# Lynne-Zheng-Linfang/HS-Pose

Hardware: AMD Instinct MI355X
Metric: point-clouds/sec (N=1028) HS-layer fwd+bwd (higher is better)
Workload: dtype f32; 1 GPU; HS stack (FaceRecon backbone -> feat) fwd+bwd, B=16/GPU N=1028 fp32, train-mode BN, random-init weights (BASELINE configs[1] shape); global_batch=16, points=1028, parallelism=dp1, hipgraph=True, split_graph=False, grad_exchange=none

## Files before the change

### hs_pose_amd/FaceRecon.py

```python
import os

import torch
import torch.nn as nn
import torch.nn.functional as F

from . import gcn3d, ops, ops_bf16, pc_sample
from .config import FLAGS


def _conv_bn_relu_rows(seq, x, n_blocks, first=None):
    if (x.dtype if x is not None else getattr(first, "dtype", None)) == torch.bfloat16:
        for i in range(n_blocks):
            conv, bn = seq[3 * i], seq[3 * i + 1]
            x = first if (i == 0 and first is not None) else ops_bf16.dense_bn(x, conv.weight.squeeze(-1), conv.bias, bn)
        return x
    for i in range(n_blocks):
        conv, bn = seq[3 * i], seq[3 * i + 1]
        y, part = first if (i == 0 and first is not None) else ops.linear_rows(x, conv.weight.squeeze(-1), conv.bias, bn_partials=True)
        x = ops.bn_relu(y, bn, partial=part)
    return x


class FaceRecon(nn.Module):

# ... 69 lines not shown
                 (w(self.face_head[6]), True, True), (w(self.face_head[9]), True, False)]
        return specs

    def forward(self, vertices: "tensor (bs, vetice_num, 3)", cat_id: "tensor (bs, 1)"):
        bs, vertice_num, _ = vertices.size()
        k = self.neighbor_num
        if self._x3 is None:
            self._x3 = ops.X3Planes()
        exact = (not self.training or self.exact_train) and self.feature_dtype == torch.float32
        with ops.x3_scope(self._x3), ops.exact_scope(exact), pc_sample.draw_scope(None, vertices.device):
            return self._forward(vertices, cat_id)

    def _forward(self, vertices, cat_id):
        bs, vertice_num, _ = vertices.size()
        k = self.neighbor_num
        if self._bf16 is not None:
            self._bf16.refresh()
        else:
            ops.x3_refresh()
        with gcn3d.knn_scope():
            up = (gcn3d.prefetch_levels(vertices, k, self.pool_1.neighbor_num, rates=(self.pool_1.pooling_rate, self.pool_2.pooling_rate),
                                        samplers=(self.pool_1.sampler, self.pool_2.sampler))
                  if self.pool_1.neighbor_num == self.pool_2.neighbor_num else None)
            od = self.feature_dtype if self.feature_dtype == torch.bfloat16 else None
            fork0 = od is None and not self.keep_backward_cut and torch.is_grad_enabled()
            if fork0:
                fm_0, a_0 = self.conv_0(vertices, k, relu_fork=True)
            else:
                fm_0 = F.relu(self.conv_0(vertices, k), inplace=True)
            fork = od is None and not self.keep_backward_cut

            def layer_bn(conv, bn, *a):
                if od is None and bn.training and bn.track_running_stats and torch.is_grad_enabled() and not ops.exact_forward():
                    out, part = conv(*a, bn_shift=True)
                    return ops.bn_relu(out, bn, fork=fork, partial=part)
                if conv is self.conv_3 and ops.exact_forward():
                    return ops.bn_relu(conv(*a, transposed_view=True), bn, out_dtype=od, fork=fork)
                return ops.bn_relu(conv(*a), bn, out_dtype=od, fork=fork)
# ... 52 lines not shown
```

### hs_pose_amd/csrc/common.h

```cpp
#pragma once
#include <hip/hip_runtime.h>
#include <stdint.h>
#include <limits.h>
#include <math.h>

#include "hsp.h"

#define HSP_WAVE 64
#define HSP_NUM_XCD 8
#define HSP_NUM_CU 256

namespace hsp {

void set_last_hip_error(hipError_t e);

inline int check_launch() {
    hipError_t e = hipGetLastError();
    if (e != hipSuccess) {
        set_last_hip_error(e);
        return HSP_ERR_LAUNCH;
    }
    return HSP_OK;
}

inline hipStream_t as_stream(hspStream_t s) { return reinterpret_cast<hipStream_t>(s); }

template <typename... P, typename... A>
inline int launch_lds(void (*kern)(P...), dim3 grid, dim3 block, size_t lds, hipStream_t st, A... args) {
    if (lds > 64 * 1024) {
        hipError_t e = hipFuncSetAttribute(reinterpret_cast<const void*>(kern), hipFuncAttributeMaxDynamicSharedMemorySize, (int)lds);
        if (e != hipSuccess) { set_last_hip_error(e); return HSP_ERR_LAUNCH; }
    }
    hipLaunchKernelGGL(kern, grid, block, lds, st, args...);
    return check_launch();
}

int knn_feat_select_flags(const float* x, int B, int N, int C, int k, int drop, int quad_mode, int32_t* idx, void* ws, size_t ws_bytes,
                          uint8_t* tie, float* dmat, hspStream_t stream);
int knn3_select_flags(const float* x, int B, int N, int k, int drop, int k2, int32_t* idx, int32_t* idx2, uint8_t* tie,
                      hipStream_t st, bool* needs_tie_pass);

int colsum_cloud_plan(int B, int N, int C, int* rows, int* nchunk);

bool orl_exact_shape_ok(int N, int C);
#define HSP_BN_MAX_PARTIALS 512
bool gemm_wave_takes(const HspGemmCall& c);
bool gemm_rows_takes(const HspGemmCall& c);

inline bool al16(const void* q, long long ld, int es) { return ((reinterpret_cast<size_t>(q) | ((size_t)ld * es)) & 15) == 0; }

inline int persistent_blocks(long long work_items, int blocks_per_cu) {
    long long g = (long long)HSP_NUM_CU * blocks_per_cu;
    if (work_items < g) g = ((work_items + HSP_NUM_XCD - 1) / HSP_NUM_XCD) * HSP_NUM_XCD;
    if (g < HSP_NUM_XCD) g = HSP_NUM_XCD;
    return (int)g;
// ... 75 lines not shown
```

### hs_pose_amd/csrc/gemm_x3.hip

```cpp
#include "common.h"
#include <stdlib.h>
#include <type_traits>

namespace hsp {

using f32x16 = __attribute__((ext_vector_type(16))) float;
using bf16x8 = __attribute__((ext_vector_type(8))) __bf16;
using u32x4 = __attribute__((ext_vector_type(4))) unsigned;

struct X3Args {
    const float* A[2];
    const unsigned short* P[2];
    int lda[2], ldp[2], K[2];
    long long ps[2];
    float* C; int ldc;
    int M, N;
    const float* bias;
    const float* resid; int ldr;
    const float* cbias; int rpc;
    float alpha;
    int tiles_m, tiles_n, nsplit;
    float* ws;
    float* bn_shift;
    float* bn_part;
// ... 441 lines not shown
            const long long row = e / N4;
            const int c4 = (int)(e - row * N4);
            *reinterpret_cast<float4*>(C + (size_t)row * ldc + 4 * c4) = make_float4(alpha * s.x, alpha * s.y, alpha * s.z, alpha * s.w);
        }
    } else {
        for (long long e = (long long)blockIdx.x * 256 + threadIdx.x; e < total; e += (long long)gridDim.x * 256) {
            float s = ws[e];
            for (int sp = 1; sp < nsplit; ++sp) s += ws[(size_t)sp * total + e];
            const long long row = e / N;
            C[(size_t)row * ldc + (int)(e - row * N)] = alpha * s;
        }
    }
}

__global__ __launch_bounds__(256) void split_params_x3_kernel(const HspSplitDesc* __restrict__ tab, int n) {
    __shared__ float tile[64][33];
    int e = 0;
    while (e + 1 < n && (int)blockIdx.x >= tab[e + 1].tile0) ++e;
    const HspSplitDesc d = tab[e];
    const int t = (int)blockIdx.x - d.tile0;
    const int Nn = d.transpose ? d.cols : d.rows, Kk = d.transpose ? d.rows : d.cols;
    const int tk = (Kk + 63) >> 6;
    const int n0 = (t / tk) * 32, k0 = (t % tk) * 64;
    const int lx = threadIdx.x & 31, ly = threadIdx.x >> 5;
    unsigned* dst = reinterpret_cast<unsigned*>(d.dst);
    float x0[4], x1[4];
    if (d.transpose) {
#pragma unroll
        for (int j = 0; j < 8; ++j) {
            const int k = k0 + ly + 8 * j, nn = n0 + lx;
            tile[ly + 8 * j][lx] = (k < Kk && nn < Nn) ? d.src[(size_t)k * d.ld + nn] : 0.f;
        }
        __syncthreads();
#pragma unroll
        for (int j = 0; j < 4; ++j) { x0[j] = tile[2 * lx][ly + 8 * j]; x1[j] = tile[2 * lx + 1][ly + 8 * j]; }
    } else {
#pragma unroll
        for (int j = 0; j < 4; ++j) {
            const int nn = n0 + ly + 8 * j, k = k0 + 2 * lx;
            const float* p = d.src + (size_t)min(nn, Nn - 1) * d.ld;
            x0[j] = (nn < Nn && k < Kk) ? p[k] : 0.f;
            x1[j] = (nn < Nn && k + 1 < Kk) ? p[k + 1] : 0.f;
        }
    }
#pragma unroll
    for (int j = 0; j < 4; ++j) {
        const int nn = n0 + ly + 8 * j, k = k0 + 2 * lx;
        if (nn >= Nn || k >= Kk) continue;
        float r1[2], r2[2];
        const float xs[2] = {x0[j], x1[j]};
#pragma unroll
        for (int q = 0; q < 2; ++q) {
            const float h = __uint_as_float(__float_as_uint(xs[q]) & 0xffff0000u);
            r1[q] = xs[q] - h;
            const float m = __uint_as_float(__float_as_uint(r1[q]) & 0xffff0000u);
            r2[q] = r1[q] - m;
        }
        const size_t o = ((size_t)nn * d.kp + k) >> 1;
        const size_t psd = (size_t)d.ps >> 1;
        dst[o] = __builtin_amdgcn_perm(__float_as_uint(xs[1]), __float_as_uint(xs[0]), 0x07060302u);
        dst[psd + o] = __builtin_amdgcn_perm(__float_as_uint(r1[1]), __float_as_uint(r1[0]), 0x07060302u);
        dst[2 * psd + o] = __builtin_amdgcn_perm(__float_as_uint(r2[1]), __float_as_uint(r2[0]), 0x07060302u);
    }
}

static int x3_pick_split(long long tiles, int TT) {
    constexpr int per_cu = 2;
    if (tiles >= 2 * HSP_NUM_CU || TT < 16) return 1;
    int ns = (int)((per_cu * HSP_NUM_CU + tiles - 1) / tiles);
    if (ns > TT / 8) ns = TT / 8;
    if (ns > 16) ns = 16;
    if (ns < 2) return 1;
    const int per = (TT + ns - 1) / ns;
    return (TT + per - 1) / per;
}

static int x3_pick_wm(int M, int N) {
    const long long t128 = (long long)((M + 127) / 128) * ((N + X3_BN - 1) / X3_BN);
// ... 504 lines not shown
```

### hs_pose_amd/csrc/knn.hip

```cpp
#include "knn_common.h"
#include "tie_pass.h"
#include <float.h>
#include <type_traits>

namespace hsp {

using f32x16 = __attribute__((ext_vector_type(16))) float;

template <int K1>
struct TopList {
    float d[K1];
    int i[K1];
    __device__ __forceinline__ void init() {
#pragma unroll
        for (int p = 0; p < K1; ++p) { d[p] = INFINITY; i[p] = INT_MAX; }
    }
    __device__ __forceinline__ void insert(float v, int idx) {
        if (v < d[K1 - 1]) {
            bool lt_cur = true;
#pragma unroll
            for (int p = K1 - 1; p > 0; --p) {
                const bool lt_prev = v < d[p - 1];
                i[p] = lt_prev ? i[p - 1] : (lt_cur ? idx : i[p]);
                d[p] = __builtin_amdgcn_fmed3f(d[p - 1], d[p], v);
// ... 296 lines not shown
                }
            }
        }
        __builtin_amdgcn_wave_barrier();
    }
}

template <int S>
__global__ __launch_bounds__(256) void knn3_wave_kernel(const float* __restrict__ x, int N, int k, int drop,
                                                        int32_t* __restrict__ idx, int msel, uint8_t* __restrict__ tie,
                                                        int msel2, int32_t* __restrict__ idx2, int k2, int tie_inline, int QW) {
    extern __shared__ __attribute__((aligned(16))) char smem[];
    const int b = blockIdx.y;
    knn3_wave_body<S>(smem, x + (size_t)b * N * 3, nullptr, nullptr, nullptr, N, k, drop, idx, msel, tie, msel2, idx2, k2, tie_inline,
                      (size_t)b * N, (int)blockIdx.x, QW);
}

template <int W>
__device__ __forceinline__ void multi_row_sum(const float* __restrict__ row, long long size, float (&out)[4][W]) {
    int lp = 0;
    {
        long long v = 1; int r = 0;
        while (v < size) { v <<= 1; ++r; }
        lp = r / 4;
        if (lp < 4) lp = 4;
    }
    const long long level_step = 1ll << lp, level_mask = level_step - 1;
    float acc[4][4][W];
#pragma unroll
    for (int a = 0; a < 4; ++a)
// ... 886 lines not shown
        default: return HSP_ERR_UNSUPPORTED;
    }
}

template <int K1, int T>
static int launch_knn3(const float* x, int B, int N, int k, int drop, int32_t* idx, hipStream_t st, int msel, uint8_t* tie,
                       int msel2, int32_t* idx2, int k2) {
    const int chunk = N < 4096 ? N : 4096;
    size_t lds = (size_t)chunk * 16;
    if (lds < (size_t)256 * K1 * 8) lds = (size_t)256 * K1 * 8;
    constexpr int Q = 256 / T;
    return launch_lds(knn3_kernel<K1, T>, dim3((N + Q - 1) / Q, B), dim3(256), lds, st, x, N, k, drop, idx, chunk, msel, tie, msel2, idx2,
                      k2);
}

static int knn3_wave_tie_inline(int N) { return N <= 64 * 9 ? 1 : 0; }

template <int S>
static int launch_knn3_wave(const float* x, int B, int N, int k, int drop, int32_t* idx, hipStream_t st, int msel, uint8_t* tie,
                            int msel2, int32_t* idx2, int k2) {
    const int tie_inline = tie ? knn3_wave_tie_inline(N) : 0;
    const size_t lds = (size_t)N * 16 + (size_t)4 * KNN3W_SV * 8 + 4 * 64 * 4 +
                       (tie_inline ? (size_t)16 * N * 4 : 0);
    const int QW = (long long)B * N >= 8192 ? KNN3W_QW : 1;
    return launch_lds(knn3_wave_kernel<S>, dim3((N + 4 * QW - 1) / (4 * QW), B), dim3(256), lds, st, x, N, k, drop, idx, msel, tie, msel2,
                      idx2, k2, tie_inline, QW);
}

template <int K1>
static int launch_knn3_t(const float* x, int B, int N, int k, int drop, int32_t* idx, hipStream_t st, int msel = 0,
                         uint8_t* tie = nullptr, int msel2 = 0, int32_t* idx2 = nullptr, int k2 = 0) {
    const long long nq = (long long)B * N;
    if (N >= 64 && (nq < 131072 || N > 64 * 17)) {
        if (N <= 64 * 5) return launch_knn3_wave<5>(x, B, N, k, drop, idx, st, msel, tie, msel2, idx2, k2);
        if (N <= 64 * 9) return launch_knn3_wave<9>(x, B, N, k, drop, idx, st, msel, tie, msel2, idx2, k2);
        if (N <= 64 * 17) return launch_knn3_wave<17>(x, B, N, k, drop, idx, st, msel, tie, msel2, idx2, k2);
        if (N <= 64 * 33) return launch_knn3_wave<33>(x, B, N, k, drop, idx, st, msel, tie, msel2, idx2, k2);
        if (N <= 64 * 65) return launch_knn3_wave<65>(x, B, N, k, drop, idx, st, msel, tie, msel2, idx2, k2);
    }
    if (nq >= 131072) return launch_knn3<K1, 1>(x, B, N, k, drop, idx, st, msel, tie, msel2, idx2, k2);
    if (nq >= 32768) return launch_knn3<K1, 4>(x, B, N, k, drop, idx, st, msel, tie, msel2, idx2, k2);
    return launch_knn3<K1, 16>(x, B, N, k, drop, idx, st, msel, tie, msel2, idx2, k2);
}

enum { KF_REM_TILE = 0,
       KF_REM_WG = 1,
       KF_REM_SYM = 2 };

static size_t knn_feat_lds(int C, int K1) {
    const int Cp = (C + 63) & ~63;
    const size_t lds = (size_t)(32 * (Cp + 4) + 4 * 32 * KF_CT_STRIDE + 4 * 32 + 32 * 8) * 4;
    const size_t lds_lists = (size_t)256 * K1 * 8;
    return lds_lists > lds ? lds_lists : lds;
}
// ... 171 lines not shown
    merge_write<K1, 2>(lists, src, ml, k, drop, ovalid, idx + ((size_t)b * N + (ovalid ? oq : 0)) * k, N, ovalid ? oq : 0);
}

template <int K1>
static int launch_knn_feat_bf16(const bf16_t* x, const float* quad, int B, int N, int C, int k, int drop, int32_t* idx,
                                hipStream_t st) {
    if (C > 256) return HSP_ERR_UNSUPPORTED;
    size_t lds = (size_t)(128 + 64) * (C * 2 + 16) + (size_t)(4 * 16 * 64 + 2 * 32 + 128 * 2) * 4;
    const size_t lds_lists = (size_t)256 * K1 * 8;
    if (lds_lists > lds) lds = lds_lists;
    if (lds > 160 * 1024) return HSP_ERR_UNSUPPORTED;
    return launch_lds(knn_feat_bf16_kernel<K1>, dim3((N + 127) / 128, B), dim3(256), lds, st, x, quad, N, C, k, drop, idx);
}

int knn3_select_flags(const float* x, int B, int N, int k, int drop, int k2, int32_t* idx, int32_t* idx2, uint8_t* tie,
                      hipStream_t st, bool* needs_tie_pass) {
    *needs_tie_pass = !(N >= 64 && (long long)B * N < 131072 && knn3_wave_tie_inline(N) != 0);
    const int m = k + drop;
    const int msel = m + 1 < N ? m + 1 : N;
    const int msel2 = k2 > 0 ? k2 + drop + 1 : 0;
    return dispatch_k1(pick_k1(msel), [&](auto K) { return launch_knn3_t<K()>(x, B, N, k, drop, idx, st, msel, tie, msel2, idx2, k2); });
}

}

using namespace hsp;

#ifdef HSP_KNN_PROF
extern "C" int hsp_debug_set_knn_prof(void* dev_buf) {
    return hipMemcpyToSymbol(HIP_SYMBOL(hsp::g_knn_prof), &dev_buf, sizeof(void*)) == hipSuccess ? 0 : -1;
}
#endif

extern "C" size_t hsp_knn_workspace_bytes(int B, int N, int C, int k) {
    (void)k;
    if (C == 3 || B <= 0 || N <= 0) return 0;
// ... 118 lines not shown
                                       int k1, int kpool, int k2, int drop_first, float* v1, float* v2, int32_t* idx1,
                                       int32_t* idx1_pool, int32_t* idx2, int32_t* up1, int32_t* up2, hspStream_t stream) {
    if (!xyz || !sel1 || !sel2 || !v1 || !v2 || !idx1 || !idx2 || !up1 || !up2 || B <= 0 || N0 <= 0 || k1 <= 0 || k2 <= 0 || kpool < 0 ||
        (kpool > 0) != (idx1_pool != nullptr) || kpool > k1)
        return HSP_ERR_BAD_ARG;
    if (!hsp_geometry_levels_takes(N0, N1, N2, k1, kpool, k2, drop_first)) return HSP_ERR_UNSUPPORTED;
    return geometry_impl(xyz, B, N0, sel1, N1, sel2, N2, k1, kpool, k2, drop_first ? 1 : 0, v1, v2, idx1, idx1_pool, idx2, up1, up2, nullptr,
                         0, 0, nullptr, nullptr, as_stream(stream));
}

extern "C" size_t hsp_geometry_all_workspace_bytes(int B, int N0) {
    if (B <= 0 || N0 <= 0) return 0;
    return ((size_t)B * N0 + 255) & ~(size_t)255;
}

extern "C" int hsp_geometry_all_f32(const float* xyz, int B, int N0, int k0, int kpool0, const int32_t* sel1, int N1,
                                    const int32_t* sel2, int N2, int k1, int kpool, int k2, int drop_first, int32_t* idx0,
                                    int32_t* idx0_pool, float* v1, float* v2, int32_t* idx1, int32_t* idx1_pool, int32_t* idx2,
                                    int32_t* up1, int32_t* up2, void* ws, size_t ws_bytes, hspStream_t stream) {
    if (!xyz || !sel1 || !sel2 || !v1 || !v2 || !idx0 || !idx1 || !idx2 || !up1 || !up2 || B <= 0 || N0 <= 0 || k0 <= 0 || k1 <= 0 ||
        k2 <= 0 || kpool < 0 || kpool0 < 0 || (kpool > 0) != (idx1_pool != nullptr) || (kpool0 > 0) != (idx0_pool != nullptr) ||
        kpool > k1 || kpool0 > k0)
        return HSP_ERR_BAD_ARG;
    const int drop = drop_first ? 1 : 0;
    if (!hsp_geometry_all_takes(B, N0, k0, kpool0, N1, N2, k1, kpool, k2, drop_first)) return HSP_ERR_UNSUPPORTED;
    if (!ws || ws_bytes < hsp_geometry_all_workspace_bytes(B, N0)) return HSP_ERR_WORKSPACE;
    uint8_t* tie = reinterpret_cast<uint8_t*>(ws);
    bool needs_pass = true;
    int rc = knn3_select_flags(xyz, B, N0, k0, drop, kpool0, idx0, idx0_pool, tie, as_stream(stream), &needs_pass);
    if (rc) return rc;
    if (!needs_pass) return HSP_ERR_UNSUPPORTED;
    return geometry_impl(xyz, B, N0, sel1, N1, sel2, N2, k1, kpool, k2, drop, v1, v2, idx1, idx1_pool, idx2, up1, up2, tie, k0, kpool0,
                         idx0, idx0_pool, as_stream(stream));
}

extern "C" int hsp_nn1_f32(const float* tgt, int Nt, const float* src, int Ns, int B, int32_t* idx,
                           hspStream_t stream) {
    if (!tgt || !src || !idx || B <= 0 || Nt <= 0 || Ns <= 0) return HSP_ERR_BAD_ARG;
    const size_t lds = (size_t)Ns * 16;
    if (lds > 160 * 1024) return HSP_ERR_UNSUPPORTED;
    return launch_lds(nn1_kernel, dim3((Nt + 255) / 256, B), dim3(256), lds, as_stream(stream), tgt, Nt, src, Ns, idx);
}
```

### hs_pose_amd/gcn3d.py

```python
import contextlib
import math

import torch
import torch.nn as nn
import torch.nn.functional as F

from . import ops, pc_sample
from .config import FLAGS

_knn_memo = None


POOL_K = 4


@contextlib.contextmanager
def knn_scope():
    global _knn_memo, _levels
    prev, _knn_memo = _knn_memo, {}
    prev_levels, _levels = _levels, None
    try:
        yield
    finally:
        _knn_memo, _levels = prev, prev_levels
# ... 26 lines not shown
    n2 = int(n1 / 4)
    k1, k2 = min(k, n1 // 8), min(k, n2 // 8)
    if (vertices.shape[2] != 3 or n2 < 1 or k1 < 1 or k2 < 1 or k1 + 1 > n1 or k2 + 1 > n2
            or not ops._takes("hsp_fps_levels_takes", n0)):
        return None
    sel1, v1, v2 = ops.fps_levels(vertices, n1, n2)
    _xyz_knn(v1, k1)
    if pool_k != POOL_K or k1 <= POOL_K:
        _xyz_knn(v1, pool_k)
    _xyz_knn(v2, k2)
    _levels = {id(vertices): (vertices, sel1, v1), id(v1): (v1, torch.arange(n2, dtype=torch.int32, device=vertices.device), v2),
               "up": (ops.nn1(vertices, v1), ops.nn1(vertices, v2))}
    return _levels["up"]


def prefetch_levels(vertices, k, pool_k=None, rates=(4, 4), samplers=(None, None)):
    global _levels
    _levels = None
    if _knn_memo is None or vertices.dtype != torch.float32 or vertices.requires_grad or not vertices.is_cuda:
        return None
    pool_k = POOL_K if pool_k is None else pool_k
    how = {resolve_sampler(s_) for s_ in samplers}
    if how != {"random"}:
        return _prefetch_levels_fps(vertices, k, pool_k) if how == {"fps"} and tuple(rates) == (4, 4) else None
    B, n0, C = vertices.shape
    n1 = int(n0 / 4)
    n2 = int(n1 / 4)
    k1, k2 = min(k, n1 // 8), min(k, n2 // 8)
    with_input = k > pool_k and ops.geometry_all_takes(B, n0, C, k, pool_k, n1, n2, k1, pool_k, k2)
    if tuple(rates) != (4, 4) or k1 <= pool_k or not (with_input or ops.geometry_levels_takes(n0, C, n1, n2, k1, pool_k, k2)):
        return None
    if _pool_feed is not None:
        sel1, sel2 = next(_pool_feed), next(_pool_feed)
        assert sel1.numel() == n1 and sel2.numel() == n2 and sel1.dtype == torch.int32
    else:
        with pc_sample.draw_scope(None, vertices.device) as device_draws:
            if device_draws is not None:
                sel1, sel2 = device_draws.pool_rows(n0, 4, levels=2)
            else:
                sel1 = torch.randperm(n0)[:n1].to(device=vertices.device, dtype=torch.int32)
                sel2 = torch.randperm(n1)[:n2].to(device=vertices.device, dtype=torch.int32)
    if with_input:
        geo = ops.geometry_all(vertices, k, pool_k, sel1, sel2, k1, pool_k, k2)
        _knn_memo[id(vertices)] = (vertices, {k: geo["idx0"], pool_k: geo["idx0_pool"]})
    else:
        geo = ops.geometry_levels(vertices, sel1, sel2, k1, pool_k, k2)
    v1, v2 = geo["v1"], geo["v2"]
    _knn_memo[id(v1)] = (v1, {k1: geo["idx1"], pool_k: geo["idx1_pool"]})
    _knn_memo[id(v2)] = (v2, {k2: geo["idx2"]})
    _levels = {id(vertices): (vertices, sel1, v1), id(v1): (v1, sel2, v2), "up": (geo["up1"], geo["up2"])}
    return _levels["up"]


def _xyz_knn(vertices, k):
    if _knn_memo is None or vertices.dtype != torch.float32:
        return ops.knn(vertices, k)
    key = id(vertices)
    hit = _knn_memo.get(key)
# ... 192 lines not shown
```

### hs_pose_amd/ops.py

```python
import ctypes
import functools
import os

import torch

from ._lib import (BATCH_SELECT_MAX_ITEMS, BATCH_SELECT_MAX_SEGS, ERR_UNSUPPORTED, FOLD_MAX_DIRS, FOLD_MAX_WGRAD, HspDirsPending, HspError,
                   HspGemmCall, HspSelectSeg, HspSplitDesc, HspWgradPending, check, lib)
from ._lib import (GEMM_BN_LINEAR as BN_LINEAR, GEMM_BN_OUT as BN_OUT, GEMM_ROUTE_SMALL_ROWS as ROUTE_SMALL_ROWS, GEMM_ROUTE_TILE as ROUTE_TILE,
                   GEMM_ROUTE_WAVE as ROUTE_WAVE, GEMM_ROUTE_X3 as ROUTE_X3, GEMM_ROUTE_X3_BN as ROUTE_X3_BN)

from .config import FLAGS

_vp = ctypes.c_void_p

DETERMINISTIC = os.environ.get("HSP_DETERMINISTIC", "0") == "1"


def _p(t):
    return _vp(t.data_ptr()) if t is not None else _vp(0)


def _stream():
    return _vp(torch.cuda.current_stream().cuda_stream)

# ... 101 lines not shown
    wsb = lib().hsp_knn_xyz_workspace_bytes(B, N)
    ws = _ws(wsb, x.device)
    _run("hsp_knn_xyz_f32", (_p(x), B, N, k, k2, 1 if drop_first else 0, _p(idx), _p(idx2), _p(ws), wsb, None, _stream()),
         key=f"B{B}N{N}k{k}", abytes=B * N * (12 + 4 * (k + k2)))
    return idx, idx2


def geometry_all_takes(B, N0, C, k0, kpool0, N1, N2, k1, kpool, k2):
    return C == 3 and 0 < kpool <= k1 and 0 < kpool0 < k0 and _takes("hsp_geometry_all_takes", B, N0, k0, kpool0, N1, N2, k1, kpool, k2, 1)


def geometry_levels_takes(N0, C, N1, N2, k1, kpool, k2):
    return C == 3 and 0 < kpool <= k1 and _takes("hsp_geometry_levels_takes", N0, N1, N2, k1, kpool, k2, 1)


def geometry_all(xyz, k0, kpool0, sel1, sel2, k1, kpool, k2):
    x = _req(xyz.detach(), torch.float32, "geometry_all.xyz")
    s1, s2 = _req(sel1, torch.int32, "geometry_all.sel1"), _req(sel2, torch.int32, "geometry_all.sel2")
    B, N0, C = x.shape
    N1, N2 = s1.numel(), s2.numel()
    if not geometry_all_takes(B, N0, C, k0, kpool0, N1, N2, k1, kpool, k2):
        return None
    dev = x.device
    i32 = dict(dtype=torch.int32, device=dev)
    out = dict(v1=torch.empty(B, N1, 3, dtype=torch.float32, device=dev), v2=torch.empty(B, N2, 3, dtype=torch.float32, device=dev),
               idx0=torch.empty(B, N0, k0, **i32), idx0_pool=torch.empty(B, N0, kpool0, **i32),
               idx1=torch.empty(B, N1, k1, **i32), idx1_pool=torch.empty(B, N1, kpool, **i32), idx2=torch.empty(B, N2, k2, **i32),
               up1=torch.empty(B, N0, **i32), up2=torch.empty(B, N0, **i32))
    wsb = lib().hsp_geometry_all_workspace_bytes(B, N0)
    ws = _ws(wsb, dev)
    _run("hsp_geometry_all_f32", (_p(x), B, N0, k0, kpool0, _p(s1), N1, _p(s2), N2, k1, kpool, k2, 1, _p(out["idx0"]), _p(out["idx0_pool"]),
                                  _p(out["v1"]), _p(out["v2"]), _p(out["idx1"]), _p(out["idx1_pool"]), _p(out["idx2"]), _p(out["up1"]),
                                  _p(out["up2"]), _p(ws), wsb, _stream()),
         key=f"B{B}N{N0}/{N1}/{N2}k{k0}", abytes=B * (12 * N0 + 4 * (N0 * (k0 + kpool0) + N1 * (k1 + kpool + 3) + N2 * (k2 + 3)) + 8 * N0))
    return out


def geometry_levels(xyz, sel1, sel2, k1, kpool, k2):
    x = _req(xyz.detach(), torch.float32, "geometry_levels.xyz")
    s1, s2 = _req(sel1, torch.int32, "geometry_levels.sel1"), _req(sel2, torch.int32, "geometry_levels.sel2")
    B, N0, C = x.shape
    N1, N2 = s1.numel(), s2.numel()
    if not geometry_levels_takes(N0, C, N1, N2, k1, kpool, k2):
        return None
    dev = x.device
    out = dict(v1=torch.empty(B, N1, 3, dtype=torch.float32, device=dev), v2=torch.empty(B, N2, 3, dtype=torch.float32, device=dev),
               idx1=torch.empty(B, N1, k1, dtype=torch.int32, device=dev), idx1_pool=torch.empty(B, N1, kpool, dtype=torch.int32, device=dev),
               idx2=torch.empty(B, N2, k2, dtype=torch.int32, device=dev), up1=torch.empty(B, N0, dtype=torch.int32, device=dev),
               up2=torch.empty(B, N0, dtype=torch.int32, device=dev))
# ... 693 lines not shown
        tab = (HspSplitDesc * len(ents))()
        tile0 = 0
        for i, e in enumerate(ents):
            W = e["src"]
            tab[i].src, tab[i].dst = W.data_ptr(), e["planes"].data_ptr()
            tab[i].rows, tab[i].cols, tab[i].ld = W.shape[0], W.shape[1], W.stride(0)
            tab[i].transpose, tab[i].kp, tab[i].tile0, tab[i].ps = int(e["transpose"]), e["kp"], tile0, e["N"] * e["kp"]
            tile0 += ((e["N"] + 31) // 32) * ((e["K"] + 63) // 64)
        return upload_table(tab, ents[0]["src"].device), tile0

    def _split(self, ents):
        tab, tiles = self._table_of(ents)
        _run("hsp_split_params_x3", (_p(tab), len(ents), tiles, _stream()), key=f"n{len(ents)}")
        return tab

    def refresh(self):
        if not self.entries:
            return
        if not self._captured and torch.cuda.is_current_stream_capturing():
            self._captured = True
        ents = list(self.entries.values())
        _run("hsp_split_params_x3", (_p(self.table), len(ents), self.total_tiles, _stream()), key=f"n{len(ents)}",
             abytes=sum(10 * e["N"] * e["K"] for e in ents))
        for e in ents:
            e["ver"] = e["src"]._version


x3_planes = X3Planes(max_entries=256)


class x3_scope:

    def __init__(self, reg):
        self.reg = reg

    def __enter__(self):
        global x3_planes
        self.prev, x3_planes = x3_planes, (self.reg if self.reg is not None else x3_planes)
        return self.reg

    def __exit__(self, *exc):
        global x3_planes
        x3_planes = self.prev
        return False


GEMM_X3 = True


def x3_refresh():
    if GEMM_X3:
        x3_planes.refresh()


def _gemm_route(A1, B1, nn1=False, A2=None, B2=None, nn2=False, bias=None, resid=None, cloud_bias=None, rows_per_cloud=0, out=None,
                alpha=1.0, xyz3=None, relu=False, bn=0):
    N = B1.shape[1] if nn1 else B1.shape[0]
    two = A2 is not None
    call = HspGemmCall(A1.data_ptr(), B1.data_ptr(), A2.data_ptr() if two else None, B2.data_ptr() if two else None,
                       resid.data_ptr() if resid is not None else None, out.data_ptr() if out is not None else None,
                       A1.shape[0], N, A1.shape[1], A2.shape[1] if two else 0, int(nn1), int(nn2), A1.element_size(),
                       _ld(A1), _ld(B1), _ld(A2) if two else 0, _ld(B2) if two else 0, _ld(resid) if resid is not None else 0,
                       _ld(out) if out is not None else N, bias is not None, cloud_bias is not None, xyz3 is not None, bool(relu),
                       alpha == 1.0, int(rows_per_cloud), bn, GEMM_X3)
    return lib().hsp_gemm_route(ctypes.byref(call))


# ... 1647 lines not shown
```

### include/hsp.h

```cpp
#ifndef HSP_H_
#define HSP_H_

#include <stddef.h>
#include <stdint.h>

#ifdef __cplusplus
extern "C" {
#endif

#define HSP_OK 0
#define HSP_ERR_BAD_ARG (-1)
#define HSP_ERR_UNSUPPORTED (-2)
#define HSP_ERR_WORKSPACE (-3)
#define HSP_ERR_LAUNCH (-4)

#define HSP_MAX_K 32

typedef void *hspStream_t;
typedef uint16_t hsp_bf16_t;

int hsp_version(void);
const char *hsp_error_string(int code);
const char *hsp_last_hip_error(void);

// ... 138 lines not shown
                       const hsp_bf16_t *A2, int lda2, const hsp_bf16_t *B2, int ldb2, int K2, int M, int N,
                       const float *bias, const hsp_bf16_t *resid, int ldr, const float *cloud_bias,
                       int rows_per_cloud, float alpha, const float *xyz3, const float *w3, void *C, int ldc,
                       int c_is_f32 ,
                       void *ws, size_t ws_bytes, hspStream_t stream);

int hsp_gemm_wave_supported(int M, int N, int K1, int K2, int cfg);
int hsp_gemm_wave_plan_info(int M, int N, int K1, int K2, int cfg, int *out);
int hsp_gemm_wave_f32(const float *A1, int lda1, const float *B1, int ldb1, int b1_layout, int K1,
                      const float *A2, int lda2, const float *B2, int ldb2, int b2_layout, int K2, int M, int N,
                      const float *bias, const float *resid, int ldr, const float *cloud_bias, int rows_per_cloud,
                      float alpha, const float *xyz3, const float *w3, float *C, int ldc, int cfg, hspStream_t stream);

typedef struct HspSplitDesc { const float *src; void *dst; int rows, cols, ld, transpose, kp, tile0; long long ps; } HspSplitDesc;
int hsp_split_params_x3(const HspSplitDesc *table_dev, int n, int total_tiles, hspStream_t stream);
int hsp_gemm_x3_supported(int M, int N, int K1, int K2);
size_t hsp_gemm_x3_workspace_bytes(int M, int N, int K1, int K2);
int hsp_gemm_x3_plan(int M, int N, int K1, int K2, int epi, int ldc, int *out);
int hsp_gemm_x3_f32(const float *A1, int lda1, const hsp_bf16_t *P1, int ldp1, long long ps1, int K1,
                    const float *A2, int lda2, const hsp_bf16_t *P2, int ldp2, long long ps2, int K2, int M, int N,
                    const float *bias, const float *resid, int ldr, const float *cloud_bias, int rows_per_cloud,
                    float alpha, float *C, int ldc, void *ws, size_t ws_bytes, hspStream_t stream);
int hsp_gemm_x3_bn_f32(const float *A1, int lda1, const hsp_bf16_t *P1, int ldp1, long long ps1, int K1,
                       const float *A2, int lda2, const hsp_bf16_t *P2, int ldp2, long long ps2, int K2, int M, int N,
                       const float *resid, int ldr, const float *cloud_bias, int rows_per_cloud, float *C, int ldc,
                       float *bn_shift, float *bn_part, hspStream_t stream);
int hsp_gemm_x3_bn_tiles(int M, int N);
int hsp_gemm_x3_bias_bn_f32(const float *A1, int lda1, const hsp_bf16_t *P1, int ldp1, long long ps1, int K1, int M, int N,
                            const float *bias, float *C, int ldc, float *bn_shift, float *bn_part, hspStream_t stream);

// ... 360 lines not shown
```

Measured before the change: 10250 point-clouds/sec.

## Fuse x3 weight-split refresh into the kNN3 wave kernel as extra blocks

Extra blocks are appended to the kNN3 wave-kernel grid to perform the bf16 three-way weight split that previously ran as its own kernel. This removes one kernel launch and lets the split overlap with the kNN search. The split body moves into a shared header, and its table lookup now uses a wave ballot instead of a serial scan. The fused path is used only for the S==17 wave variant with random sampling and geometry_all; every other case falls back to the separate refresh. A failed fused launch returns an error rather than falling back.

After: 10320 point-clouds/sec, median of 6. No clear change (+0.7%).

```diff
diff --git a/hs_pose_amd/FaceRecon.py b/hs_pose_amd/FaceRecon.py
--- a/hs_pose_amd/FaceRecon.py
+++ b/hs_pose_amd/FaceRecon.py
@@ -107,14 +107,18 @@
     def _forward(self, vertices, cat_id):
         bs, vertice_num, _ = vertices.size()
         k = self.neighbor_num
+        one_k = self.pool_1.neighbor_num == self.pool_2.neighbor_num
+        rider = None
         if self._bf16 is not None:
             self._bf16.refresh()
         else:
-            ops.x3_refresh()
+            rider = ops.x3_rider() if one_k else None
+            if rider is None:
+                ops.x3_refresh()
         with gcn3d.knn_scope():
             up = (gcn3d.prefetch_levels(vertices, k, self.pool_1.neighbor_num, rates=(self.pool_1.pooling_rate, self.pool_2.pooling_rate),
-                                        samplers=(self.pool_1.sampler, self.pool_2.sampler))
-                  if self.pool_1.neighbor_num == self.pool_2.neighbor_num else None)
+                                        samplers=(self.pool_1.sampler, self.pool_2.sampler), split=rider)
+                  if one_k else None)
             od = self.feature_dtype if self.feature_dtype == torch.bfloat16 else None
             fork0 = od is None and not self.keep_backward_cut and torch.is_grad_enabled()
             if fork0:
diff --git a/hs_pose_amd/csrc/common.h b/hs_pose_amd/csrc/common.h
--- a/hs_pose_amd/csrc/common.h
+++ b/hs_pose_amd/csrc/common.h
@@ -38,7 +38,8 @@
 int knn_feat_select_flags(const float* x, int B, int N, int C, int k, int drop, int quad_mode, int32_t* idx, void* ws, size_t ws_bytes,
                           uint8_t* tie, float* dmat, hspStream_t stream);
 int knn3_select_flags(const float* x, int B, int N, int k, int drop, int k2, int32_t* idx, int32_t* idx2, uint8_t* tie,
-                      hipStream_t st, bool* needs_tie_pass);
+                      hipStream_t st, bool* needs_tie_pass, const HspSplitDesc* split_tab = nullptr, int split_n = 0,
+                      int split_tiles = 0);
 
 int colsum_cloud_plan(int B, int N, int C, int* rows, int* nchunk);
 
diff --git a/hs_pose_amd/csrc/gemm_x3.hip b/hs_pose_amd/csrc/gemm_x3.hip
--- a/hs_pose_amd/csrc/gemm_x3.hip
+++ b/hs_pose_amd/csrc/gemm_x3.hip
@@ -1,4 +1,5 @@
 #include "common.h"
+#include "split_x3.h"
 #include <stdlib.h>
 #include <type_traits>
 
@@ -479,54 +480,8 @@
 }
 
 __global__ __launch_bounds__(256) void split_params_x3_kernel(const HspSplitDesc* __restrict__ tab, int n) {
-    __shared__ float tile[64][33];
-    int e = 0;
-    while (e + 1 < n && (int)blockIdx.x >= tab[e + 1].tile0) ++e;
-    const HspSplitDesc d = tab[e];
-    const int t = (int)blockIdx.x - d.tile0;
-    const int Nn = d.transpose ? d.cols : d.rows, Kk = d.transpose ? d.rows : d.cols;
-    const int tk = (Kk + 63) >> 6;
-    const int n0 = (t / tk) * 32, k0 = (t % tk) * 64;
-    const int lx = threadIdx.x & 31, ly = threadIdx.x >> 5;
-    unsigned* dst = reinterpret_cast<unsigned*>(d.dst);
-    float x0[4], x1[4];
-    if (d.transpose) {
-#pragma unroll
-        for (int j = 0; j < 8; ++j) {
-            const int k = k0 + ly + 8 * j, nn = n0 + lx;
-            tile[ly + 8 * j][lx] = (k < Kk && nn < Nn) ? d.src[(size_t)k * d.ld + nn] : 0.f;
-        }
-        __syncthreads();
-#pragma unroll
-        for (int j = 0; j < 4; ++j) { x0[j] = tile[2 * lx][ly + 8 * j]; x1[j] = tile[2 * lx + 1][ly + 8 * j]; }
-    } else {
-#pragma unroll
-        for (int j = 0; j < 4; ++j) {
-            const int nn = n0 + ly + 8 * j, k = k0 + 2 * lx;
-            const float* p = d.src + (size_t)min(nn, Nn - 1) * d.ld;
-            x0[j] = (nn < Nn && k < Kk) ? p[k] : 0.f;
-            x1[j] = (nn < Nn && k + 1 < Kk) ? p[k + 1] : 0.f;
-        }
-    }
-#pragma unroll
-    for (int j = 0; j < 4; ++j) {
-        const int nn = n0 + ly + 8 * j, k = k0 + 2 * lx;
-        if (nn >= Nn || k >= Kk) continue;
-        float r1[2], r2[2];
-        const float xs[2] = {x0[j], x1[j]};
-#pragma unroll
-        for (int q = 0; q < 2; ++q) {
-            const float h = __uint_as_float(__float_as_uint(xs[q]) & 0xffff0000u);
-            r1[q] = xs[q] - h;
-            const float m = __uint_as_float(__float_as_uint(r1[q]) & 0xffff0000u);
-            r2[q] = r1[q] - m;
-        }
-        const size_t o = ((size_t)nn * d.kp + k) >> 1;
-        const size_t psd = (size_t)d.ps >> 1;
-        dst[o] = __builtin_amdgcn_perm(__float_as_uint(xs[1]), __float_as_uint(xs[0]), 0x07060302u);
-        dst[psd + o] = __builtin_amdgcn_perm(__float_as_uint(r1[1]), __float_as_uint(r1[0]), 0x07060302u);
-        dst[2 * psd + o] = __builtin_amdgcn_perm(__float_as_uint(r2[1]), __float_as_uint(r2[0]), 0x07060302u);
-    }
+    __shared__ float tile[SPLIT_X3_TILE_FLOATS];
+    split_params_x3_body(tab, n, (int)blockIdx.x, tile);
 }
 
 static int x3_pick_split(long long tiles, int TT) {
diff --git a/hs_pose_amd/csrc/knn.hip b/hs_pose_amd/csrc/knn.hip
--- a/hs_pose_amd/csrc/knn.hip
+++ b/hs_pose_amd/csrc/knn.hip
@@ -1,5 +1,6 @@
 #include "knn_common.h"
 #include "tie_pass.h"
+#include "split_x3.h"
 #include <float.h>
 #include <type_traits>
 
@@ -334,6 +335,24 @@
     const int b = blockIdx.y;
     knn3_wave_body<S>(smem, x + (size_t)b * N * 3, nullptr, nullptr, nullptr, N, k, drop, idx, msel, tie, msel2, idx2, k2, tie_inline,
                       (size_t)b * N, (int)blockIdx.x, QW);
+}
+
+template <int S>
+__global__ __launch_bounds__(256) void knn3_wave_split_kernel(const float* __restrict__ x, int N, int k, int drop,
+                                                              int32_t* __restrict__ idx, int msel, uint8_t* __restrict__ tie,
+                                                              int msel2, int32_t* __restrict__ idx2, int k2, int tie_inline, int QW,
+                                                              int qcols, const HspSplitDesc* __restrict__ tab, int ntab,
+                                                              int total_tiles) {
+    extern __shared__ __attribute__((aligned(16))) char smem[];
+    const int lin = (int)blockIdx.x + (int)gridDim.x * (int)blockIdx.y, nsearch = qcols * (int)gridDim.y;
+    if (lin >= nsearch) {
+        const int piece = lin - nsearch;
+        if (piece < total_tiles) split_params_x3_body(tab, ntab, piece, reinterpret_cast<float*>(smem));
+        return;
+    }
+    const int b = lin / qcols;
+    knn3_wave_body<S>(smem, x + (size_t)b * N * 3, nullptr, nullptr, nullptr, N, k, drop, idx, msel, tie, msel2, idx2, k2, tie_inline,
+                      (size_t)b * N, lin - b * qcols, QW);
 }
 
 template <int W>
@@ -1250,30 +1269,44 @@
                       k2);
 }
 
+struct SplitRider { const HspSplitDesc* tab; int n, tiles; };
+
 static int knn3_wave_tie_inline(int N) { return N <= 64 * 9 ? 1 : 0; }
 
 template <int S>
 static int launch_knn3_wave(const float* x, int B, int N, int k, int drop, int32_t* idx, hipStream_t st, int msel, uint8_t* tie,
-                            int msel2, int32_t* idx2, int k2) {
+                            int msel2, int32_t* idx2, int k2, const SplitRider& rider) {
     const int tie_inline = tie ? knn3_wave_tie_inline(N) : 0;
     const size_t lds = (size_t)N * 16 + (size_t)4 * KNN3W_SV * 8 + 4 * 64 * 4 +
                        (tie_inline ? (size_t)16 * N * 4 : 0);
     const int QW = (long long)B * N >= 8192 ? KNN3W_QW : 1;
+    if (rider.tab) {
+        if constexpr (S == 17) {
+            if (lds < SPLIT_X3_TILE_FLOATS * sizeof(float)) return HSP_ERR_UNSUPPORTED;
+            const int qcols = (N + 4 * QW - 1) / (4 * QW);
+            return launch_lds(knn3_wave_split_kernel<S>, dim3(qcols + (rider.tiles + B - 1) / B, B), dim3(256), lds, st, x, N, k, drop, idx,
+                              msel, tie, msel2, idx2, k2, tie_inline, QW, qcols, rider.tab, rider.n, rider.tiles);
+        } else {
+            return HSP_ERR_UNSUPPORTED;
+        }
+    }
     return launch_lds(knn3_wave_kernel<S>, dim3((N + 4 * QW - 1) / (4 * QW), B), dim3(256), lds, st, x, N, k, drop, idx, msel, tie, msel2,
                       idx2, k2, tie_inline, QW);
 }
 
 template <int K1>
 static int launch_knn3_t(const float* x, int B, int N, int k, int drop, int32_t* idx, hipStream_t st, int msel = 0,
-                         uint8_t* tie = nullptr, int msel2 = 0, int32_t* idx2 = nullptr, int k2 = 0) {
+                         uint8_t* tie = nullptr, int msel2 = 0, int32_t* idx2 = nullptr, int k2 = 0,
+                         const SplitRider& rider = SplitRider{nullptr, 0, 0}) {
     const long long nq = (long long)B * N;
     if (N >= 64 && (nq < 131072 || N > 64 * 17)) {
-        if (N <= 64 * 5) return launch_knn3_wave<5>(x, B, N, k, drop, idx, st, msel, tie, msel2, idx2, k2);
-        if (N <= 64 * 9) return launch_knn3_wave<9>(x, B, N, k, drop, idx, st, msel, tie, msel2, idx2, k2);
-        if (N <= 64 * 17) return launch_knn3_wave<17>(x, B, N, k, drop, idx, st, msel, tie, msel2, idx2, k2);
-        if (N <= 64 * 33) return launch_knn3_wave<33>(x, B, N, k, drop, idx, st, msel, tie, msel2, idx2, k2);
-        if (N <= 64 * 65) return launch_knn3_wave<65>(x, B, N, k, drop, idx, st, msel, tie, msel2, idx2, k2);
-    }
+        if (N <= 64 * 5) return launch_knn3_wave<5>(x, B, N, k, drop, idx, st, msel, tie, msel2, idx2, k2, rider);
+        if (N <= 64 * 9) return launch_knn3_wave<9>(x, B, N, k, drop, idx, st, msel, tie, msel2, idx2, k2, rider);
+        if (N <= 64 * 17) return launch_knn3_wave<17>(x, B, N, k, drop, idx, st, msel, tie, msel2, idx2, k2, rider);
+        if (N <= 64 * 33) return launch_knn3_wave<33>(x, B, N, k, drop, idx, st, msel, tie, msel2, idx2, k2, rider);
+        if (N <= 64 * 65) return launch_knn3_wave<65>(x, B, N, k, drop, idx, st, msel, tie, msel2, idx2, k2, rider);
+    }
+    if (rider.tab) return HSP_ERR_UNSUPPORTED;
     if (nq >= 131072) return launch_knn3<K1, 1>(x, B, N, k, drop, idx, st, msel, tie, msel2, idx2, k2);
     if (nq >= 32768) return launch_knn3<K1, 4>(x, B, N, k, drop, idx, st, msel, tie, msel2, idx2, k2);
     return launch_knn3<K1, 16>(x, B, N, k, drop, idx, st, msel, tie, msel2, idx2, k2);
@@ -1475,12 +1508,13 @@
 }
 
 int knn3_select_flags(const float* x, int B, int N, int k, int drop, int k2, int32_t* idx, int32_t* idx2, uint8_t* tie,
-                      hipStream_t st, bool* needs_tie_pass) {
+                      hipStream_t st, bool* needs_tie_pass, const HspSplitDesc* split_tab, int split_n, int split_tiles) {
     *needs_tie_pass = !(N >= 64 && (long long)B * N < 131072 && knn3_wave_tie_inline(N) != 0);
     const int m = k + drop;
     const int msel = m + 1 < N ? m + 1 : N;
     const int msel2 = k2 > 0 ? k2 + drop + 1 : 0;
-    return dispatch_k1(pick_k1(msel), [&](auto K) { return launch_knn3_t<K()>(x, B, N, k, drop, idx, st, msel, tie, msel2, idx2, k2); });
+    const SplitRider rider{split_tab, split_n, split_tiles};
+    return dispatch_k1(pick_k1(msel), [&](auto K) { return launch_knn3_t<K()>(x, B, N, k, drop, idx, st, msel, tie, msel2, idx2, k2, rider); });
 }
 
 }
@@ -1629,10 +1663,10 @@
     return ((size_t)B * N0 + 255) & ~(size_t)255;
 }
 
-extern "C" int hsp_geometry_all_f32(const float* xyz, int B, int N0, int k0, int kpool0, const int32_t* sel1, int N1,
-                                    const int32_t* sel2, int N2, int k1, int kpool, int k2, int drop_first, int32_t* idx0,
-                                    int32_t* idx0_pool, float* v1, float* v2, int32_t* idx1, int32_t* idx1_pool, int32_t* idx2,
-                                    int32_t* up1, int32_t* up2, void* ws, size_t ws_bytes, hspStream_t stream) {
+static int geometry_all_impl(const float* xyz, int B, int N0, int k0, int kpool0, const int32_t* sel1, int N1, const int32_t* sel2, int N2,
+                             int k1, int kpool, int k2, int drop_first, int32_t* idx0, int32_t* idx0_pool, float* v1, float* v2,
+                             int32_t* idx1, int32_t* idx1_pool, int32_t* idx2, int32_t* up1, int32_t* up2, void* ws, size_t ws_bytes,
+                             hspStream_t stream, const HspSplitDesc* split_tab, int split_n, int split_tiles) {
     if (!xyz || !sel1 || !sel2 || !v1 || !v2 || !idx0 || !idx1 || !idx2 || !up1 || !up2 || B <= 0 || N0 <= 0 || k0 <= 0 || k1 <= 0 ||
         k2 <= 0 || kpool < 0 || kpool0 < 0 || (kpool > 0) != (idx1_pool != nullptr) || (kpool0 > 0) != (idx0_pool != nullptr) ||
         kpool > k1 || kpool0 > k0)
@@ -1642,11 +1676,30 @@
     if (!ws || ws_bytes < hsp_geometry_all_workspace_bytes(B, N0)) return HSP_ERR_WORKSPACE;
     uint8_t* tie = reinterpret_cast<uint8_t*>(ws);
     bool needs_pass = true;
-    int rc = knn3_select_flags(xyz, B, N0, k0, drop, kpool0, idx0, idx0_pool, tie, as_stream(stream), &needs_pass);
+    int rc = knn3_select_flags(xyz, B, N0, k0, drop, kpool0, idx0, idx0_pool, tie, as_stream(stream), &needs_pass, split_tab, split_n,
+                               split_tiles);
     if (rc) return rc;
     if (!needs_pass) return HSP_ERR_UNSUPPORTED;
     return geometry_impl(xyz, B, N0, sel1, N1, sel2, N2, k1, kpool, k2, drop, v1, v2, idx1, idx1_pool, idx2, up1, up2, tie, k0, kpool0,
                          idx0, idx0_pool, as_stream(stream));
+}
+
+extern "C" int hsp_geometry_all_f32(const float* xyz, int B, int N0, int k0, int kpool0, const int32_t* sel1, int N1,
+                                    const int32_t* sel2, int N2, int k1, int kpool, int k2, int drop_first, int32_t* idx0,
+                                    int32_t* idx0_pool, float* v1, float* v2, int32_t* idx1, int32_t* idx1_pool, int32_t* idx2,
+                                    int32_t* up1, int32_t* up2, void* ws, size_t ws_bytes, hspStream_t stream) {
+    return geometry_all_impl(xyz, B, N0, k0, kpool0, sel1, N1, sel2, N2, k1, kpool, k2, drop_first, idx0, idx0_pool, v1, v2, idx1, idx1_pool,
+                             idx2, up1, up2, ws, ws_bytes, stream, nullptr, 0, 0);
+}
+
+extern "C" int hsp_geometry_all_split_f32(const float* xyz, int B, int N0, int k0, int kpool0, const int32_t* sel1, int N1,
+                                          const int32_t* sel2, int N2, int k1, int kpool, int k2, int drop_first, int32_t* idx0,
+                                          int32_t* idx0_pool, float* v1, float* v2, int32_t* idx1, int32_t* idx1_pool, int32_t* idx2,
+                                          int32_t* up1, int32_t* up2, void* ws, size_t ws_bytes, hspStream_t stream,
+                                          const HspSplitDesc* table_dev, int n, int total_tiles) {
+    if (!table_dev || n <= 0 || total_tiles <= 0) return HSP_ERR_BAD_ARG;
+    return geometry_all_impl(xyz, B, N0, k0, kpool0, sel1, N1, sel2, N2, k1, kpool, k2, drop_first, idx0, idx0_pool, v1, v2, idx1, idx1_pool,
+                             idx2, up1, up2, ws, ws_bytes, stream, table_dev, n, total_tiles);
 }
 
 extern "C" int hsp_nn1_f32(const float* tgt, int Nt, const float* src, int Ns, int B, int32_t* idx,
diff --git a/hs_pose_amd/csrc/split_x3.h b/hs_pose_amd/csrc/split_x3.h
--- /dev/null
+++ b/hs_pose_amd/csrc/split_x3.h
@@ -0,0 +1,64 @@
+#pragma once
+#include "common.h"
+
+namespace hsp {
+
+#define SPLIT_X3_TILE_FLOATS (64 * 33)
+
+__device__ __forceinline__ void split_params_x3_body(const HspSplitDesc* __restrict__ tab, int n, int piece, float* __restrict__ tile) {
+    const int lane = threadIdx.x & 63;
+    int cnt = 0;
+    for (int i0 = 0; i0 < n; i0 += 64) {
+        const int i = i0 + lane;
+        const bool le = i < n && tab[i].tile0 <= piece;
+        cnt += __popcll(__ballot(le));
+    }
+    const int e = __builtin_amdgcn_readfirstlane(cnt > 0 ? cnt - 1 : 0);
+    const HspSplitDesc d = tab[e];
+    const int t = piece - d.tile0;
+    const int Nn = d.transpose ? d.cols : d.rows, Kk = d.transpose ? d.rows : d.cols;
+    const int tk = (Kk + 63) >> 6;
+    const int n0 = (t / tk) * 32, k0 = (t % tk) * 64;
+    const int lx = threadIdx.x & 31, ly = threadIdx.x >> 5;
+    unsigned* dst = reinterpret_cast<unsigned*>(d.dst);
+    float x0[4], x1[4];
+    if (d.transpose) {
+#pragma unroll
+        for (int j = 0; j < 8; ++j) {
+            const int k = k0 + ly + 8 * j, nn = n0 + lx;
+            tile[(ly + 8 * j) * 33 + lx] = (k < Kk && nn < Nn) ? d.src[(size_t)k * d.ld + nn] : 0.f;
+        }
+        __syncthreads();
+#pragma unroll
+        for (int j = 0; j < 4; ++j) { x0[j] = tile[2 * lx * 33 + ly + 8 * j]; x1[j] = tile[(2 * lx + 1) * 33 + ly + 8 * j]; }
+    } else {
+#pragma unroll
+        for (int j = 0; j < 4; ++j) {
+            const int nn = n0 + ly + 8 * j, k = k0 + 2 * lx;
+            const float* p = d.src + (size_t)min(nn, Nn - 1) * d.ld;
+            x0[j] = (nn < Nn && k < Kk) ? p[k] : 0.f;
+            x1[j] = (nn < Nn && k + 1 < Kk) ? p[k + 1] : 0.f;
+        }
+    }
+#pragma unroll
+    for (int j = 0; j < 4; ++j) {
+        const int nn = n0 + ly + 8 * j, k = k0 + 2 * lx;
+        if (nn >= Nn || k >= Kk) continue;
+        float r1[2], r2[2];
+        const float xs[2] = {x0[j], x1[j]};
+#pragma unroll
+        for (int q = 0; q < 2; ++q) {
+            const float h = __uint_as_float(__float_as_uint(xs[q]) & 0xffff0000u);
+            r1[q] = xs[q] - h;
+            const float m = __uint_as_float(__float_as_uint(r1[q]) & 0xffff0000u);
+            r2[q] = r1[q] - m;
+        }
+        const size_t o = ((size_t)nn * d.kp + k) >> 1;
+        const size_t psd = (size_t)d.ps >> 1;
+        dst[o] = __builtin_amdgcn_perm(__float_as_uint(xs[1]), __float_as_uint(xs[0]), 0x07060302u);
+        dst[psd + o] = __builtin_amdgcn_perm(__float_as_uint(r1[1]), __float_as_uint(r1[0]), 0x07060302u);
+        dst[2 * psd + o] = __builtin_amdgcn_perm(__float_as_uint(r2[1]), __float_as_uint(r2[0]), 0x07060302u);
+    }
+}
+
+}
diff --git a/hs_pose_amd/gcn3d.py b/hs_pose_amd/gcn3d.py
--- a/hs_pose_amd/gcn3d.py
+++ b/hs_pose_amd/gcn3d.py
@@ -64,14 +64,21 @@
     return _levels["up"]
 
 
-def prefetch_levels(vertices, k, pool_k=None, rates=(4, 4), samplers=(None, None)):
+def prefetch_levels(vertices, k, pool_k=None, rates=(4, 4), samplers=(None, None), split=None):
     global _levels
     _levels = None
+
+    def no_ride():
+        if split is not None:
+            split.refresh()
+
     if _knn_memo is None or vertices.dtype != torch.float32 or vertices.requires_grad or not vertices.is_cuda:
+        no_ride()
         return None
     pool_k = POOL_K if pool_k is None else pool_k
     how = {resolve_sampler(s_) for s_ in samplers}
     if how != {"random"}:
+        no_ride()
         return _prefetch_levels_fps(vertices, k, pool_k) if how == {"fps"} and tuple(rates) == (4, 4) else None
     B, n0, C = vertices.shape
     n1 = int(n0 / 4)
@@ -79,7 +86,10 @@
     k1, k2 = min(k, n1 // 8), min(k, n2 // 8)
     with_input = k > pool_k and ops.geometry_all_takes(B, n0, C, k, pool_k, n1, n2, k1, pool_k, k2)
     if tuple(rates) != (4, 4) or k1 <= pool_k or not (with_input or ops.geometry_levels_takes(n0, C, n1, n2, k1, pool_k, k2)):
+        no_ride()
         return None
+    if not with_input:
+        no_ride()
     if _pool_feed is not None:
         sel1, sel2 = next(_pool_feed), next(_pool_feed)
         assert sel1.numel() == n1 and sel2.numel() == n2 and sel1.dtype == torch.int32
@@ -91,7 +101,8 @@
                 sel1 = torch.randperm(n0)[:n1].to(device=vertices.device, dtype=torch.int32)
                 sel2 = torch.randperm(n1)[:n2].to(device=vertices.device, dtype=torch.int32)
     if with_input:
-        geo = ops.geometry_all(vertices, k, pool_k, sel1, sel2, k1, pool_k, k2)
+        geo = (ops.geometry_all(vertices, k, pool_k, sel1, sel2, k1, pool_k, k2) if split is None else
+               ops.geometry_all(vertices, k, pool_k, sel1, sel2, k1, pool_k, k2, split=split))
         _knn_memo[id(vertices)] = (vertices, {k: geo["idx0"], pool_k: geo["idx0_pool"]})
     else:
         geo = ops.geometry_levels(vertices, sel1, sel2, k1, pool_k, k2)
diff --git a/hs_pose_amd/ops.py b/hs_pose_amd/ops.py
--- a/hs_pose_amd/ops.py
+++ b/hs_pose_amd/ops.py
@@ -139,7 +139,7 @@
     return C == 3 and 0 < kpool <= k1 and _takes("hsp_geometry_levels_takes", N0, N1, N2, k1, kpool, k2, 1)
 
 
-def geometry_all(xyz, k0, kpool0, sel1, sel2, k1, kpool, k2):
+def geometry_all(xyz, k0, kpool0, sel1, sel2, k1, kpool, k2, split=None):
     x = _req(xyz.detach(), torch.float32, "geometry_all.xyz")
     s1, s2 = _req(sel1, torch.int32, "geometry_all.sel1"), _req(sel2, torch.int32, "geometry_all.sel2")
     B, N0, C = x.shape
@@ -154,10 +154,15 @@
                up1=torch.empty(B, N0, **i32), up2=torch.empty(B, N0, **i32))
     wsb = lib().hsp_geometry_all_workspace_bytes(B, N0)
     ws = _ws(wsb, dev)
-    _run("hsp_geometry_all_f32", (_p(x), B, N0, k0, kpool0, _p(s1), N1, _p(s2), N2, k1, kpool, k2, 1, _p(out["idx0"]), _p(out["idx0_pool"]),
-                                  _p(out["v1"]), _p(out["v2"]), _p(out["idx1"]), _p(out["idx1_pool"]), _p(out["idx2"]), _p(out["up1"]),
-                                  _p(out["up2"]), _p(ws), wsb, _stream()),
-         key=f"B{B}N{N0}/{N1}/{N2}k{k0}", abytes=B * (12 * N0 + 4 * (N0 * (k0 + kpool0) + N1 * (k1 + kpool + 3) + N2 * (k2 + 3)) + 8 * N0))
+    args = (_p(x), B, N0, k0, kpool0, _p(s1), N1, _p(s2), N2, k1, kpool, k2, 1, _p(out["idx0"]), _p(out["idx0_pool"]), _p(out["v1"]),
+            _p(out["v2"]), _p(out["idx1"]), _p(out["idx1_pool"]), _p(out["idx2"]), _p(out["up1"]), _p(out["up2"]), _p(ws), wsb, _stream())
+    ab = B * (12 * N0 + 4 * (N0 * (k0 + kpool0) + N1 * (k1 + kpool + 3) + N2 * (k2 + 3)) + 8 * N0)
+    if split is not None:
+        table, n, tiles = split.ride()
+        _run("hsp_geometry_all_split_f32", args + (_p(table), n, tiles), key=f"B{B}N{N0}/{N1}/{N2}k{k0}+n{n}",
+             abytes=ab + split.split_bytes())
+    else:
+        _run("hsp_geometry_all_f32", args, key=f"B{B}N{N0}/{N1}/{N2}k{k0}", abytes=ab)
     return out
 
 
@@ -881,16 +886,23 @@
         _run("hsp_split_params_x3", (_p(tab), len(ents), tiles, _stream()), key=f"n{len(ents)}")
         return tab
 
+    def split_bytes(self):
+        return sum(10 * e["N"] * e["K"] for e in self.entries.values())
+
+    def ride(self):
+        if not self.entries:
+            raise HspError("X3Planes.ride: an empty registry has no split to hand over")
+        if not self._captured and torch.cuda.is_current_stream_capturing():
+            self._captured = True
+        for e in self.entries.values():
+            e["ver"] = e["src"]._version
+        return self.table, len(self.entries), self.total_tiles
+
     def refresh(self):
         if not self.entries:
             return
-        if not self._captured and torch.cuda.is_current_stream_capturing():
-            self._captured = True
-        ents = list(self.entries.values())
-        _run("hsp_split_params_x3", (_p(self.table), len(ents), self.total_tiles, _stream()), key=f"n{len(ents)}",
-             abytes=sum(10 * e["N"] * e["K"] for e in ents))
-        for e in ents:
-            e["ver"] = e["src"]._version
+        table, n, tiles = self.ride()
+        _run("hsp_split_params_x3", (_p(table), n, tiles, _stream()), key=f"n{n}", abytes=self.split_bytes())
 
 
 x3_planes = X3Planes(max_entries=256)
@@ -918,6 +930,13 @@
 def x3_refresh():
     if GEMM_X3:
         x3_planes.refresh()
+
+
+SPLIT_RIDER = os.environ.get("HSP_SPLIT_RIDER", "1") != "0"
+
+
+def x3_rider():
+    return x3_planes if GEMM_X3 and SPLIT_RIDER and x3_planes.entries else None
 
 
 def _gemm_route(A1, B1, nn1=False, A2=None, B2=None, nn2=False, bias=None, resid=None, cloud_bias=None, rows_per_cloud=0, out=None,
diff --git a/include/hsp.h b/include/hsp.h
--- a/include/hsp.h
+++ b/include/hsp.h
@@ -176,6 +176,10 @@
 
 typedef struct HspSplitDesc { const float *src; void *dst; int rows, cols, ld, transpose, kp, tile0; long long ps; } HspSplitDesc;
 int hsp_split_params_x3(const HspSplitDesc *table_dev, int n, int total_tiles, hspStream_t stream);
+int hsp_geometry_all_split_f32(const float *xyz, int B, int N0, int k0, int kpool0, const int32_t *sel1, int N1, const int32_t *sel2,
+                               int N2, int k1, int kpool, int k2, int drop_first, int32_t *idx0, int32_t *idx0_pool, float *v1,
+                               float *v2, int32_t *idx1, int32_t *idx1_pool, int32_t *idx2, int32_t *up1, int32_t *up2, void *ws,
+                               size_t ws_bytes, hspStream_t stream, const HspSplitDesc *table_dev, int n, int total_tiles);
 int hsp_gemm_x3_supported(int M, int N, int K1, int K2);
 size_t hsp_gemm_x3_workspace_bytes(int M, int N, int K1, int K2);
 int hsp_gemm_x3_plan(int M, int N, int K1, int K2, int epi, int ldc, int *out);
```
